# KikeM/romtime

Hardware: AMD Instinct MI355X
Metric: snapshot-DoF/s for POD build (higher is better)
Workload: dtype f64

## Files before the change

include/romtime_hip.h:

```cpp
#ifndef ROMTIME_HIP_H
#define ROMTIME_HIP_H

#include <stdint.h>

#ifdef __cplusplus
extern "C" {
#endif

typedef struct rt_ctx rt_ctx;

#define RT_OK 0
#define RT_ERR_ARG (-1)
#define RT_ERR_HIP (-2)
#define RT_ERR_UNSUPPORTED (-3)
#define RT_WARN_ZERO_NORM 1
#define RT_WARN_SINGULAR 2

#define RT_ROW_MAJOR 0
#define RT_COL_MAJOR 1

int rt_version(void);
int rt_ctx_create(rt_ctx** out, int device);
void rt_ctx_destroy(rt_ctx* ctx);
int rt_ctx_set_stream(rt_ctx* ctx, void* hip_stream);
// ... 113 lines not shown

int rt_trajectory_errors(rt_ctx* ctx, const double* B, int64_t ldb, const double* A, int64_t lda, int64_t stride_a,
                         const double* U, int64_t ldu, int u_layout, int64_t stride_u, int64_t N, int64_t k, int64_t nt,
                         int64_t n_traj, double* err, double* ref);

#define RT_FN_POWER 0
int rt_trajectory_integrals(rt_ctx* ctx, const double* E, int64_t lde, const double* w, const double* A, int64_t lda,
                            int64_t stride_a, const double* scale, int64_t n_pts, int64_t k, int64_t nt, int64_t n_traj,
                            int fn, const double* par, double* out);
int rt_trajectory_integrals_plan_info(int num_cus, const double* E, int64_t lde, const double* w, const double* A, int64_t lda,
                                      int64_t stride_a, const double* scale, int64_t n_pts, int64_t k, int64_t nt,
                                      int64_t n_traj, int fn, const double* par, const double* out, int64_t* info3);

int rt_interpolation_errors(rt_ctx* ctx, const double* Psi, int64_t ldpsi, const int64_t* idx, int64_t m, const double* F,
                            int64_t ldf, int f_layout, int64_t N, int64_t S, int64_t group, int64_t pin_row, double pin_value,
                            double* err, double* ref);
int rt_interpolation_errors_plan_info(int num_cus, const double* Psi, int64_t ldpsi, const int64_t* idx, int64_t m,
                                      const double* F, int64_t ldf, int f_layout, int64_t N, int64_t S, int64_t group,
                                      int64_t pin_row, double pin_value, const double* err, const double* ref, int64_t* info3);

#define RT_P1_MASS 0
#define RT_P1_STIFFNESS 1
#define RT_P1_CONVECTION 2
#define RT_P1_TRILINEAR 3
#define RT_P1_LOAD 4
#define RT_P1_LOAD_P2 5
int rt_p1_local_assembly(rt_ctx* ctx, int kind, int64_t nx, const int64_t* rows, const int64_t* cols, int64_t m,
                         int64_t n_states, const double* h, const double* coef, int state_mode, const double* state,
                         double* out);

int rt_sym_eig_values(rt_ctx* ctx, const double* G, int64_t n, double* lam, int* status);
int rt_sym_eig_values_part(rt_ctx* ctx, const double* G, int64_t n, int64_t first, int64_t count, double* lam,
                           int* status);
int rt_sym_eig_vectors(rt_ctx* ctx, int64_t n, int64_t k, const double* lam, double* W);

int rt_sym_jacobi_eigh(rt_ctx* ctx, const double* A, int64_t n, double* lam, double* W, int max_sweeps, int* sweeps_done,
                       int* status);

int rt_host_jacobi_eigh(double* A, int64_t n, double* W, double* lam, int max_sweeps, int* sweeps_done);

int rt_bench_mfma_f64(rt_ctx* ctx, int iters, double* tflops);
int rt_bench_copy(rt_ctx* ctx, void* dst, const void* src, int64_t bytes, int reps, double* gbps);

#ifdef __cplusplus
}
#endif
#endif
```

romtime_amd/_lib.py:

```python
from __future__ import annotations

import ctypes as C
import os
import threading
import weakref

_HERE = os.path.dirname(os.path.abspath(__file__))
LIB_PATH = os.path.join(_HERE, "lib", "libromtime_hip.so")

ROW_MAJOR, COL_MAJOR = 0, 1
RT_OK = 0
WARN_ZERO_NORM, WARN_SINGULAR = 1, 2

_p = C.c_void_p
_i64 = C.c_int64
_int = C.c_int

SOLVER_DIRECT, SOLVER_GMRES = 0, 1


class GmresOpts(C.Structure):

    _fields_ = [("rtol", C.c_double), ("atol", C.c_double), ("restart", _i64), ("maxiter", _i64)]

# ... 17 lines not shown
    "rt_last_sweep_stats": (_int, [_p, C.POINTER(_i64)]),
    "rt_gram": (_int, [_p, _p, _i64, _i64, _i64, _int, _p]),
    "rt_gram_scale": (_int, [_p, _p, _i64, _p, _int, _p]),
    "rt_pod_backproject_weights": (_int, [_p, _p, _i64, _i64, _p, _p, _p]),
    "rt_pod_enqueue": (_int, [_p, _p, _i64, _i64, _i64, _int, _i64, _int, _p, _p, _p, _p, _p, _p, _p]),
    "rt_pod_orth": (_int, [_p, _p, _i64, _i64, _i64, _int, _i64, C.c_double, _int, _p, _i64, C.POINTER(_i64), _p, _p,
                           C.POINTER(_int)]),
    "rt_gemm_tn": (_int, [_p, _p, _i64, _int, _p, _i64, _int, _i64, _i64, _i64, _p, _i64]),
    "rt_gemm_nn": (_int, [_p, _p, _i64, _int, _p, _i64, _i64, _i64, _i64, _p, _i64, _int]),
    "rt_rank_update": (_int, [_p, _p, _i64, _p, _p, _i64, _p, _i64, _i64, _i64, _i64, C.c_double, _p, _i64]),
    "rt_gemm_nn_axpby": (_int, [_p, _p, _i64, _int, _p, _i64, _i64, _i64, _i64, C.c_double, C.c_double, _p, _i64, _int]),
    "rt_transpose": (_int, [_p, _p, _i64, _i64, _i64, _p, _i64]),
    "rt_deim_greedy": (_int, [_p, _p, _i64, _i64, _i64, _int, _p, _p, _p]),
    "rt_csr_spmm": (_int, [_p, _p, _p, _p, _i64, _p, _i64, _i64, _p, _i64]),
    "rt_project_csr": (_int, [_p, _p, _p, _p, _i64, _p, _i64, _i64, _p]),
    "rt_project_csr_batched": (_int, [_p, _p, _p, _p, _i64, _int, _i64, _i64, _p, _i64, _i64, _p]),
    "rt_dense_solve_batched": (_int, [_p, _p, _p, _i64, _i64, _p]),
    "rt_dense_solve_multi": (_int, [_p, _p, _i64, _p, _p, _i64, _p]),
    "rt_tracked_solve_batched": (_int, [_p, _p, _p, _p, _i64, _i64, _int, _p]),
    "rt_gmres_batched": (_int, [_p, _p, _p, _p, _i64, _i64, C.POINTER(GmresOpts), _p, _p]),
    "rt_ctx_set_reduced_solver": (_int, [_p, _int, C.POINTER(GmresOpts)]),
    "rt_rom_bdf_sweep": (_int, [_p, _p, _p]),
    "rt_hrom_bdf_sweep": (_int, [_p, _p, _p]),
    "rt_trajectory_errors": (_int, [_p, _p, _i64, _p, _i64, _i64, _p, _i64, _int, _i64, _i64, _i64, _i64, _i64, _p, _p]),
    "rt_trajectory_integrals": (_int, [_p, _p, _i64, _p, _p, _i64, _i64, _p, _i64, _i64, _i64, _i64, _int, C.POINTER(C.c_double), _p]),
    "rt_trajectory_integrals_plan_info": (_int, [_int, _p, _i64, _p, _p, _i64, _i64, _p, _i64, _i64, _i64, _i64, _int,
                                                 C.POINTER(C.c_double), _p, C.POINTER(_i64)]),
    "rt_interpolation_errors": (_int, [_p, _p, _i64, C.POINTER(_i64), _i64, _p, _i64, _int, _i64, _i64, _i64, _i64, C.c_double, _p, _p]),
    "rt_interpolation_errors_plan_info": (_int, [_int, _p, _i64, C.POINTER(_i64), _i64, _p, _i64, _int, _i64, _i64, _i64, _i64,
                                                 C.c_double, _p, _p, C.POINTER(_i64)]),
    "rt_p1_local_assembly": (_int, [_p, _int, _i64, _p, _p, _i64, _i64, _p, _p, _int, _p, _p]),
    "rt_sym_eig_values": (_int, [_p, _p, _i64, _p, _p]),
    "rt_sym_eig_values_part": (_int, [_p, _p, _i64, _i64, _i64, _p, _p]),
    "rt_sym_eig_vectors": (_int, [_p, _i64, _i64, _p, _p]),
    "rt_sym_jacobi_eigh": (_int, [_p, _p, _i64, _p, _p, _int, C.POINTER(_int), _p]),
    "rt_host_jacobi_eigh": (_int, [_p, _i64, _p, _p, _int, C.POINTER(_int)]),
    "rt_bench_mfma_f64": (_int, [_p, _int, C.POINTER(C.c_double)]),
    "rt_bench_copy": (_int, [_p, _p, _p, _i64, _int, C.POINTER(C.c_double)]),
}



class SweepDesc(C.Structure):

    _fields_ = [("N", _i64), ("nnz", _i64), ("r", _i64), ("n_mu", _i64), ("nt", _i64), ("dt", C.c_double),
                ("bdf2", _int), ("indptr", _p), ("indices", _p), ("V", _p), ("mass_values", _p), ("n_terms", _i64),
                ("term_values", _p), ("term_coef", _p), ("tril_values", _p), ("n_rhs", _i64), ("rhs_terms", _p),
                ("rhs_coef", _p)]


class HSweepDesc(C.Structure):

    _fields_ = [("r", _i64), ("n_mu", _i64), ("nt", _i64), ("dt", C.c_double), ("bdf2", _int), ("m_mass", _i64),
                ("m_lin", _i64), ("m_nl", _i64), ("m_rhs", _i64), ("Z", _p), ("Zf", _p), ("F_mass", _p), ("F_lin", _p),
                ("F_rhs", _p), ("W", _p), ("C_nl", _p), ("S_nl", _p)]


_lib = None
_lock = threading.Lock()


class RomtimeHipError(RuntimeError):
    pass


def load():
# ... 156 lines not shown
```

romtime_amd/csrc/api.hip:

```cpp
#include "common.h"

#include <chrono>
#include <new>

namespace {

int grow(rt_ctx* ctx, void** buf, size_t* have, size_t bytes, void** out) {
  if (bytes > *have) {
    RT_HIP_CHECK(ctx, hipStreamSynchronize(ctx->stream));
    if (*buf) RT_HIP_CHECK(ctx, hipFree(*buf));
    *buf = nullptr;
    *have = 0;
    const size_t want = (bytes + ((size_t)1 << 20) - 1) & ~(((size_t)1 << 20) - 1);
    RT_HIP_CHECK(ctx, hipMalloc(buf, want));
    *have = want;
  }
  *out = *buf;
  return RT_OK;
}

__global__ void gram_scale_kernel(double* __restrict__ G, int n, double* __restrict__ colnorm, int normalize,
                                  int* status_flag) {
  const long idx = (long)blockIdx.x * blockDim.x + threadIdx.x;
  if (idx >= (long)n * n) return;
// ... 123 lines not shown
  for (const void* f : ctx->lds_done)
    if (f == fn) return RT_OK;
  RT_HIP_CHECK(ctx, hipFuncSetAttribute(fn, hipFuncAttributeMaxDynamicSharedMemorySize, bytes));
  ctx->lds_done.push_back(fn);
  return RT_OK;
}

int rt_profile_begin(rt_ctx* ctx, bool also_gram) {
  if (!ctx->profile) return RT_OK;
  if (!ctx->ev0) {
    RT_HIP_CHECK(ctx, hipEventCreate(&ctx->ev0));
    RT_HIP_CHECK(ctx, hipEventCreate(&ctx->ev1));
  }
  if (also_gram && !ctx->gev0) {
    RT_HIP_CHECK(ctx, hipEventCreate(&ctx->gev0));
    RT_HIP_CHECK(ctx, hipEventCreate(&ctx->gev1));
  }
  RT_HIP_CHECK(ctx, hipEventRecord(ctx->ev0, ctx->stream));
  if (also_gram) RT_HIP_CHECK(ctx, hipEventRecord(ctx->gev0, ctx->stream));
  return RT_OK;
}

int rt_profile_end(rt_ctx* ctx, bool also_gram) {
  if (!ctx->profile) return RT_OK;
  RT_HIP_CHECK(ctx, hipEventRecord(ctx->ev1, ctx->stream));
  if (also_gram) RT_HIP_CHECK(ctx, hipEventRecord(ctx->gev1, ctx->stream));
  ctx->ev_valid = true;
  if (also_gram) ctx->gev_valid = true;
  return RT_OK;
}

extern "C" {

int rt_version(void) { return 380; }

int rt_ctx_create(rt_ctx** out, int device) {
  if (!out) return RT_ERR_ARG;
  *out = nullptr;
  int count = 0;
  if (hipGetDeviceCount(&count) != hipSuccess || device < 0 || device >= count) return RT_ERR_HIP;
  if (hipSetDevice(device) != hipSuccess) return RT_ERR_HIP;
  rt_ctx* ctx = new (std::nothrow) rt_ctx();
  if (!ctx) return RT_ERR_HIP;
  ctx->device = device;
  hipDeviceProp_t prop;
  if (hipGetDeviceProperties(&prop, device) == hipSuccess) ctx->num_cus = ctx->device_cus = prop.multiProcessorCount;
  if (hipMalloc(reinterpret_cast<void**>(&ctx->dev_counters), sizeof(long) * RT_N_COUNTERS) != hipSuccess ||
      hipMemset(ctx->dev_counters, 0, sizeof(long) * RT_N_COUNTERS) != hipSuccess) {
    delete ctx;
    return RT_ERR_HIP;
  }
  *out = ctx;
  return RT_OK;
}

void rt_ctx_destroy(rt_ctx* ctx) {
  if (!ctx) return;
  (void)hipSetDevice(ctx->device);
  (void)hipDeviceSynchronize();
  if (ctx->scratch) (void)hipFree(ctx->scratch);
  if (ctx->scratch2) (void)hipFree(ctx->scratch2);
  if (ctx->dev_counters) (void)hipFree(ctx->dev_counters);
  if (ctx->gram_pace) (void)hipFree(ctx->gram_pace);
  if (ctx->ev0) (void)hipEventDestroy(ctx->ev0);
  if (ctx->ev1) (void)hipEventDestroy(ctx->ev1);
  if (ctx->gev0) (void)hipEventDestroy(ctx->gev0);
  if (ctx->gev1) (void)hipEventDestroy(ctx->gev1);
// ... 292 lines not shown
```

romtime_amd/csrc/symeig.hip:

```cpp
#include <type_traits>

#include "common.h"
#include "wave_ops.h"

namespace {

constexpr int TW_SMALL = 32;
constexpr int SLOT0 = 160;
constexpr int TW_LARGE = 128;
constexpr int LPR = 64;
constexpr int TT = 1024;
static_assert(LPR == 64, "row reductions use the whole-wave DPP sum");
constexpr int NMAX = 1024;
constexpr int VEC_ITERS = 2;

struct TriParams {
  const double* G;
  double* V;
  double* P;
  double* tau;
  double* d;
  double* e;
  int* flags;
  int n;
// ... 282 lines not shown
      if (gi > k && gi < n) {
        double* row = A + (size_t)li * n;
        const double vi = sv[gi], wi = sw[gi];
        for (int j = k + 1 + tx; j < n; j += LPR) row[j] -= vi * sw[j] + wi * sv[j];
      }
    }
  }
  __syncthreads();
  if (wg == (n - 2) % TW && tid == 0) {
    p.d[n - 2] = sl[n - 2];
    p.e[n - 2] = sl[n - 1];
  }
  if (wg == (n - 1) % TW && tid == 0) {
    p.d[n - 1] = A[(size_t)((n - 1) / TW) * lda + (n - 1)];
    p.e[n - 1] = 0.0;
  }
}

__device__ __forceinline__ double fast_rcp(double q) {
  const double r = __builtin_amdgcn_rcp(q);
  return fma(fma(-q, r, 1.0), r, r);
}

__global__ void symeig_init_kernel(int* flags, double* tau, int n) {
  for (int i = threadIdx.x; i < SLOT0 + TW_LARGE; i += blockDim.x) flags[i] = 0;
  for (int i = threadIdx.x; i < n; i += blockDim.x) tau[i] = 0.0;
}

constexpr int BIS_NS = 2;
template <int NM>
__global__ __launch_bounds__(256) void symeig_bisect_kernel(const double* __restrict__ d, const double* __restrict__ e,
                                                            int n, int first, int count, double* __restrict__ lam,
                                                            const int* flags, int* status, long* counters) {
  if (blockIdx.x == 0 && threadIdx.x == 0) {
    if (status) *status = flags[3];
    if (flags[3]) atomicAdd(reinterpret_cast<unsigned long long*>(&counters[RT_CNT_EIG_TIMEOUT]), 1ull);
  }
  __shared__ double sd[NM], se2[NM];
  __shared__ int s_first[2][4];
  const int tid = threadIdx.x, lane = tid & 63, wid = tid >> 6, half = wid & 1;
  double glo = 1e300, ghi = -1e300, emax = 0.0;
  for (int i = lane; i < n; i += 64) {
    const double di = d[i], ei = (i + 1 < n) ? e[i] : 0.0, el = (i > 0) ? fabs(e[i - 1]) : 0.0;
    sd[i] = di;
    se2[i] = ei * ei;
    glo = fmin(glo, di - el - fabs(ei));
    ghi = fmax(ghi, di + el + fabs(ei));
    emax = fmax(emax, ei * ei);
  }
  glo = rtw::wave_min(glo);
  ghi = rtw::wave_max(ghi);
  emax = rtw::wave_max(emax);
  __syncthreads();
  const double tn = fmax(fabs(glo), fabs(ghi));
  double lo = glo - 2.2e-16 * tn * n - 1e-300, hi = ghi + 2.2e-16 * tn * n + 1e-300;
  const double pivmin = 2.2250738585072014e-308 * fmax(1.0, emax);
  const int j = first + min(2 * (int)blockIdx.x + (wid >> 1), count - 1);
  const int want = n - j;
  constexpr int NSH = 128 * BIS_NS;
  constexpr int NSEC = NSH + 1;
  for (int pass = 0; pass < 7; ++pass) {
    const double h = (hi - lo) / NSEC;
    const int s0 = BIS_NS * (64 * half + lane);
    const double x0 = lo + h * (s0 + 1), x1 = x0 + h;
    double q0 = sd[0] - x0, q1 = sd[0] - x1;
    if (fabs(q0) < pivmin) q0 = -pivmin;
    if (fabs(q1) < pivmin) q1 = -pivmin;
// ... 364 lines not shown
        p.d[n - 1] = p.A[(size_t)(n - 1) * lda + (n - 1)] - (v[q] * w[q] + w[q] * v[q]);
      }
  }
}
static_assert(NWIDE % WIDE_CHUNK == 0 && NWIDE % WIDE_T == 0, "the reflector kernel covers a padded row with PER elements per thread");

template <int LO, int HI, class F>
int size_class(int64_t n, F&& f) {
  if constexpr (LO < HI)
    if (n > LO) return size_class<2 * LO, HI>(n, f);
  return f(std::integral_constant<int, LO>{});
}

struct EigArena {
  void* base;
  double *V, *own, *tau, *d, *e;
  int* flags;
  int carve(rt_ctx* ctx, int64_t n, size_t own_bytes) {
    rt_carver a;
    const size_t oV = a.add(sizeof(double) * n * n), oO = a.add(own_bytes), oT = a.add(sizeof(double) * n),
                 oD = a.add(sizeof(double) * n), oE = a.add(sizeof(double) * n), oF = a.add(sizeof(int) * (SLOT0 + TW_LARGE));
    RT_TRY(rt_scratch2(ctx, a.total(), &base));
    V = a.at<double>(base, oV); own = a.at<double>(base, oO);
    tau = a.at<double>(base, oT); d = a.at<double>(base, oD);
    e = a.at<double>(base, oE); flags = a.at<int>(base, oF);
    return RT_OK;
  }
  void publish(rt_ctx* ctx, int64_t n) const {
    ctx->eig.d = d; ctx->eig.e = e; ctx->eig.V = V; ctx->eig.tau = tau; ctx->eig.n = n; ctx->eig.base = base;
    ctx->eig.gen = ctx->scratch2_gen;
  }
};

int launch_bisect(rt_ctx* ctx, const EigArena& a, int64_t n, int64_t first, int64_t count, double* lam, int* status) {
  return size_class<512, NWIDE>(n, [&](auto nm) {
    hipLaunchKernelGGL(symeig_bisect_kernel<decltype(nm)::value>, dim3((unsigned)((count + 1) / 2)), dim3(256), 0, ctx->stream, a.d,
                       a.e, (int)n, (int)first, (int)count, lam, a.flags, status, ctx->dev_counters);
    RT_HIP_CHECK(ctx, hipGetLastError());
    return (int)RT_OK;
  });
}

}

static int sym_eig_values_wide(rt_ctx* ctx, const double* G, int64_t n, int64_t first, int64_t count, double* lam,
                               int* status) {
  const int lda = (int)((n + WIDE_CHUNK - 1) / WIDE_CHUNK * WIDE_CHUNK);
  const size_t nvec = (size_t)3 * (lda + WIDE_ROWS) + (size_t)(n + WIDE_ROWS);
  static_assert(sizeof(double) * WIDE_CHUNK % 256 == 0, "the vector buffers start on a 256-byte boundary");
  const size_t cells = (size_t)(n + WIDE_ROWS) * lda;
  EigArena ar;
  RT_TRY(ar.carve(ctx, n, sizeof(double) * (cells + nvec)));
  WideParams wp;
  wp.V = ar.V; wp.A = ar.own;
  wp.vb = wp.A + cells; wp.w = wp.vb + (size_t)2 * (lda + WIDE_ROWS);
  wp.pr = wp.w + (lda + WIDE_ROWS);
  wp.tau = ar.tau; wp.d = ar.d; wp.e = ar.e;
  wp.n = (int)n; wp.lda = lda; wp.counters = ctx->dev_counters;
  hipStream_t st = ctx->stream;
  hipLaunchKernelGGL(symeig_init_kernel, dim3(1), dim3(256), 0, st, ar.flags, wp.tau, (int)n);
  hipLaunchKernelGGL(symeig_wide_load_kernel, dim3((unsigned)((cells + WIDE_T - 1) / WIDE_T)), dim3(WIDE_T), 0, st, G, wp,
                     (long)nvec);
  hipLaunchKernelGGL(symeig_wide_reflect_kernel, dim3(1), dim3(WIDE_T), 0, st, wp, -1);
  RT_HIP_CHECK(ctx, hipGetLastError());
  for (int k = 0; k + 2 < (int)n; ++k) {
    const int rows = (int)n - 1 - k;
    hipLaunchKernelGGL(symeig_wide_sweep_kernel, dim3((unsigned)((rows + WIDE_ROWS - 1) / WIDE_ROWS)), dim3(WIDE_T), 0, st, wp, k);
    hipLaunchKernelGGL(symeig_wide_reflect_kernel, dim3(1), dim3(WIDE_T), 0, st, wp, k);
  }
  RT_HIP_CHECK(ctx, hipGetLastError());
  RT_TRY(launch_bisect(ctx, ar, n, first, count, lam, status));
  ar.publish(ctx, n);
  return RT_OK;
}

extern "C" int rt_sym_eig_values(rt_ctx* ctx, const double* G, int64_t n, double* lam, int* status) {
  return rt_sym_eig_values_part(ctx, G, n, 0, n, lam, status);
}

extern "C" int rt_sym_eig_values_part(rt_ctx* ctx, const double* G, int64_t n, int64_t first, int64_t count, double* lam,
                                      int* status) {
  if (!ctx) return RT_ERR_ARG;
  RT_ARG_CHECK(ctx, G && lam && n >= 3 && first >= 0 && count >= 1 && first + count <= n);
  if (n > NWIDE) {
    ctx->err = "rt_sym_eig_values: n > 2048 not supported (the limit of the device eigensolver)";
    return RT_ERR_UNSUPPORTED;
  }
  if (n > NMAX) return sym_eig_values_wide(ctx, G, n, first, count, lam, status);
  const bool large = n > 512;
  const bool small_team = !large && ctx->num_cus < TW_SMALL && ctx->num_cus >= TW_SMALL / 2;
  int tw = large ? TW_LARGE : (small_team ? TW_SMALL / 2 : TW_SMALL);
  const bool local = n <= 64;
  if (local) tw = 1;
  if (tw > ctx->num_cus) {
    ctx->err = "rt_sym_eig_values: not enough compute units for the cooperative tridiagonalisation";
    return RT_ERR_UNSUPPORTED;
  }
  EigArena ar;
  RT_TRY(ar.carve(ctx, n, sizeof(double) * 4 * n));
  TriParams tp;
  tp.G = G; tp.n = (int)n; tp.tw = tw;
  tp.spread = (!large && !local && ctx->eig_one_xcd && ctx->num_cus / 8 >= tw) ? 1 : 0;
  tp.local = local ? 1 : 0;
  tp.xcd = ctx->eig_xcd & 7;
  tp.V = ar.V; tp.P = ar.own; tp.tau = ar.tau; tp.d = ar.d; tp.e = ar.e; tp.flags = ar.flags;
  tp.counters = ctx->dev_counters;
  hipStream_t st = ctx->stream;
  hipLaunchKernelGGL(symeig_init_kernel, dim3(1), dim3(256), 0, st, tp.flags, tp.tau, (int)n);

  const int RB = (int)((n + tw - 1) / tw);
  const size_t lds = sizeof(double) * ((size_t)RB * (local ? n + 2 : n) + 5 * n + 16);
  const auto tridiag = [&](auto nm) -> int {
    const auto kernel = &symeig_tridiag_kernel<decltype(nm)::value>;
    RT_TRY(rt_func_lds(ctx, reinterpret_cast<const void*>(kernel), 150 * 1024));
    int per_cu = 0;
    RT_HIP_CHECK(ctx, hipOccupancyMaxActiveBlocksPerMultiprocessor(&per_cu, kernel, TT, lds));
    if ((long)per_cu * ctx->num_cus < tw) {
      ctx->err = "rt_sym_eig_values: the device cannot keep all cooperating workgroups resident";
      return RT_ERR_UNSUPPORTED;
    }
    hipLaunchKernelGGL(kernel, dim3(tp.spread ? 16 * tw : tw), dim3(TT), lds, st, tp);
    RT_HIP_CHECK(ctx, hipGetLastError());
    return RT_OK;
  };
  RT_TRY((size_class<128, NMAX>(n, tridiag)));
  RT_TRY(launch_bisect(ctx, ar, n, first, count, lam, status));
  ar.publish(ctx, n);
  return RT_OK;
}

extern "C" int rt_sym_eig_vectors(rt_ctx* ctx, int64_t n, int64_t k, const double* lam, double* W) {
  if (!ctx) return RT_ERR_ARG;
  RT_ARG_CHECK(ctx, lam && W && k >= 1 && k <= n);
  if (ctx->eig.n != n || ctx->eig.base == nullptr || ctx->eig.base != ctx->scratch2 || ctx->eig.gen != ctx->scratch2_gen) {
    ctx->err = "rt_sym_eig_vectors: must follow rt_sym_eig_values on the same ctx and matrix with no other composite "
               "operator (greedy, projection, sweep) in between";
    return RT_ERR_ARG;
  }
  VecParams vp;
  vp.d = ctx->eig.d; vp.e = ctx->eig.e; vp.lam = lam; vp.V = ctx->eig.V; vp.tau = ctx->eig.tau;
  vp.W = W; vp.n = (int)n; vp.k = (int)k;
  const int nblk = (int)((n - 2 + RBK - 1) / RBK);
  void* cbuf = nullptr;
  int rc = rt_scratch(ctx, sizeof(double) * 6 * (size_t)nblk, &cbuf);
  if (rc != RT_OK) return rc;
  vp.C = static_cast<const double*>(cbuf);
  return size_class<128, NWIDE>(n, [&](auto nm) -> int {
    constexpr int NM = decltype(nm)::value;
    const size_t vlds = sizeof(double) * (8 * NM + 8) + NM;
    RT_TRY(rt_func_lds(ctx, reinterpret_cast<const void*>(&symeig_vectors_kernel<NM>), (NM > 1024 ? 136 : 80) * 1024));
    hipLaunchKernelGGL(symeig_wy_kernel<NM>, dim3((unsigned)nblk), dim3(64), 0, ctx->stream, vp.V, (int)n,
                       static_cast<double*>(cbuf));
    hipLaunchKernelGGL(symeig_vectors_kernel<NM>, dim3((unsigned)k), dim3(64), vlds, ctx->stream, vp);
    RT_HIP_CHECK(ctx, hipGetLastError());
    return RT_OK;
  });
}
```

romtime_amd/ops.py:

```python
from __future__ import annotations

import ctypes as C

import numpy as np
import torch

from . import _lib, pod_rules
from ._lib import COL_MAJOR, ROW_MAJOR, Context, RomtimeHipError

_p = C.c_void_p


def _ptr(t):
    return _p(t.data_ptr()) if t is not None else _p(None)


def _need_gpu():
    if not torch.cuda.is_available():
        raise RomtimeHipError("no MI355X visible: romtime_amd's hot path runs on the GPU only (there is no CPU fallback)")


def to_device(a, device=None) -> torch.Tensor:
    _need_gpu()
    if isinstance(a, torch.Tensor):
# ... 378 lines not shown
    mode, st = 0, None
    if state is not None:
        st = to_device(state).contiguous()
        width = 2 * nx + 1 if kind == "load_p2" else nx + 1
        if tuple(st.shape) != (n_states, width):
            raise RomtimeHipError(f"p1_local_assembly: `state` must be (n_states, {width}) for kind {kind!r}")
        mode = 1
    elif ramp is not None:
        st = to_device(np.atleast_1d(ramp) if not isinstance(ramp, torch.Tensor) else ramp).contiguous()
        mode = 2
    elif poly is not None:
        st = to_device(poly).contiguous()
        if tuple(st.shape) != (n_states, 3):
            raise RomtimeHipError("p1_local_assembly: `poly` must be (n_states, 3)")
        mode = 3
    out = torch.empty((n_states, m), dtype=torch.float64, device=h.device)
    ctx.check(ctx.lib.rt_p1_local_assembly(ctx.handle, P1_KINDS[kind], int(nx), _ptr(rows), _ptr(cols), m, n_states, _ptr(h),
                                           _ptr(coef), mode, _ptr(st), _ptr(out)), "rt_p1_local_assembly")
    return out


def sym_eig_values(G: torch.Tensor, first: int = 0, count: int | None = None):
    ctx = Context.current()
    n = G.shape[0]
    assert G.is_contiguous() and G.shape == (n, n)
    count = n - first if count is None else count
    lam = torch.empty(n, dtype=torch.float64, device=G.device)
    status = torch.zeros(1, dtype=torch.int32, device=G.device)
    ctx.check(ctx.lib.rt_sym_eig_values_part(ctx.handle, _ptr(G), n, first, count, _ptr(lam), _ptr(status)),
              "rt_sym_eig_values_part")
    return lam, status


def sym_eig_vectors(lam: torch.Tensor, k: int, first: int = 0) -> torch.Tensor:
    ctx = Context.current()
    n = lam.numel()
    W = torch.empty((n, k), dtype=torch.float64, device=lam.device)
    ctx.check(ctx.lib.rt_sym_eig_vectors(ctx.handle, n, k, _ptr(lam[first:]), _ptr(W)), "rt_sym_eig_vectors")
    return W


def sym_jacobi_eigh(G: torch.Tensor, max_sweeps: int = 60):
    ctx = Context.current()
    n = G.shape[0]
    if G.dtype != torch.float64 or not G.is_cuda or G.dim() != 2 or G.shape != (n, n):
        raise RomtimeHipError("sym_jacobi_eigh: expected a square float64 CUDA tensor")
    G = G.contiguous()
    lam = torch.empty(n, dtype=torch.float64, device=G.device)
    W = torch.empty((n, n), dtype=torch.float64, device=G.device)
    status = torch.zeros(1, dtype=torch.int32, device=G.device)
    sweeps = C.c_int(0)
    ctx.check(ctx.lib.rt_sym_jacobi_eigh(ctx.handle, _ptr(G), n, _ptr(lam), _ptr(W), int(max_sweeps), C.byref(sweeps),
                                         _ptr(status)), "rt_sym_jacobi_eigh")
    if sweeps.value >= max_sweeps and int(status.item()) != 0:
        import warnings

        warnings.warn(f"romtime_amd: sym_jacobi_eigh stopped at max_sweeps = {max_sweeps} with rotations still applied",
                      RuntimeWarning)
    return lam, W, int(sweeps.value)


def transpose(src: torch.Tensor) -> torch.Tensor:
    ctx = Context.current()
    src = src.contiguous()
    rows, cols = src.shape
    dst = torch.empty((cols, rows), dtype=torch.float64, device=src.device)
# ... 19 lines not shown
```

romtime_amd/pipeline.py:

```python
from __future__ import annotations

import collections
import ctypes as C
import os
import weakref

import torch

from . import _lib, ops, pod, pod_rules

_p = C.c_void_p


SMALL_SET = 150_000_000
_STREAMS: dict = {}
_STREAMS_PID: list = []
_OPEN_RUNS = weakref.WeakSet()


def shutdown():
    import gc

    if not _STREAMS:
        return
    if _STREAMS_PID and _STREAMS_PID[0] != os.getpid():
        _STREAMS.clear()
        return
    try:
        for gen in list(_OPEN_RUNS):
            gen.close()
        torch.cuda.synchronize()
        gc.collect()
        torch.cuda.empty_cache()
        lib = _lib.load()
        _lib.Context.unbind_streams()
        for st in list(_STREAMS.values()):
            lib.rt_stream_destroy(_p(st.cuda_stream))
    finally:
        _STREAMS.clear()


def _masked_stream(lib, dev, first, count):
    key = (dev, first, count)
    if key not in _STREAMS:
        h = _p()
        rc = lib.rt_stream_create_cu_range(dev, first, count, C.byref(h))
        if rc != 0:
# ... 66 lines not shown
    def _gram(self, item):
        X = item["X"]
        n = X.shape[1]
        with self.ctxG.use(self.sG):
            item["t0"] = torch.cuda.Event(enable_timing=True)
            item["t0"].record()
            Gbuf = torch.empty(n * n + 1, dtype=torch.float64, device=X.device)
            item["G"] = ops.gram(X, out=Gbuf[: n * n].view(n, n))
            Gbuf[n * n:].fill_(float(X.shape[0]))
            item["k0"] = torch.cuda.Event(enable_timing=True)
            item["k0"].record()
            item["Gbuf"] = Gbuf
        st = self.sG if self.sR is None else self.sR
        with torch.cuda.stream(st):
            if st is not self.sG:
                st.wait_event(item["k0"])
            if self.group is not None:
                import torch.distributed as dist

                dist.all_reduce(Gbuf, op=dist.ReduceOp.SUM, group=self.group)
            item["g"] = torch.cuda.Event(enable_timing=True)
            item["g"].record()

    def _eig(self, item):
        k, normalize = item["k"], item["normalize"]
        item["owner"] = item["index"] % self.world
        if self.rank != item["owner"]:
            return
        with self.ctxE.use(self.sE):
            self.sE.wait_event(item["g"])
            G = item["G"]
            n = G.shape[0]
            colnorm, flag = ops.gram_scale(G, normalize)
            lam_d, status = ops.sym_eig_values(G)
            Z = ops.sym_eig_vectors(lam_d, k)
            Zs = ops.backproject_weights(Z, lam_d, colnorm if normalize else None)
            item["payload"] = torch.cat([lam_d, colnorm, status.to(torch.float64), flag.to(torch.float64), Zs.reshape(-1)])
            item["_keep"] = (lam_d, status, flag, Z, Zs, colnorm)
            item["ec"] = torch.cuda.Event(enable_timing=True)
            item["ec"].record()

    def _share(self, item):
        n, k = item["G"].shape[0], item["k"]
        st = self.sE if self.group_e is None else self.sC
        with torch.cuda.stream(st):
            if self.group_e is not None:
                import torch.distributed as dist

                if self.rank == item["owner"]:
                    st.wait_event(item["ec"])
                else:
                    item["payload"] = torch.empty(n * (k + 2) + 2, dtype=torch.float64, device=item["G"].device)
                dist.broadcast(item["payload"], src=dist.get_global_rank(self.group_e, item["owner"]), group=self.group_e)
            payload = item["payload"]
            item["colnorm"].copy_(payload[n:2 * n])
            item["Zs"] = payload[2 * n + 2:].view(n, k)
            head = pod.pack_head(payload[:n], payload[2 * n:2 * n + 2], item["Gbuf"][-1:])
            item["head"] = torch.empty(head.numel(), dtype=torch.float64).pin_memory()
            item["head"].copy_(head, non_blocking=True)
            item["_keep2"] = head
            item["e"] = torch.cuda.Event(enable_timing=True)
            item["e"].record()

    def _backproject(self, item):
        ctx, st = self.ctxG, self.sG
        with ctx.use(st):
            st.wait_event(item["e"])
            ops.gemm_nn(item["X"], item["Zs"], out=item["Q"])
            item["b"] = torch.cuda.Event(enable_timing=True)
            item["b"].record()

    def _regular(self, item):
        self.recomputed += 1
        self.sE.synchronize()
        return pod.pod_device(item["X"], num=item["num"], normalize=item["normalize"], group=self.group)

    def _finish(self, item):
        if item["direct"]:
            return self._regular(item)
        item["b"].synchronize()
        head = pod_rules.parse_head(item["head"].numpy(), item["X"].shape[1])
        if item["normalize"] and head.zero_norm:
            raise pod_rules.zero_norm_error()
        r = pod_rules.single_pass_rank(head.lam, head.status, head.n_rows, item["k"], num=item["num"])
        self.last_stage_ms = dict(gram_kernel_ms=item["t0"].elapsed_time(item["k0"]),
                                  gram_allreduce_ms=item["t0"].elapsed_time(item["g"]),
                                  eig_chain_ms=item["g"].elapsed_time(item["e"]),
                                  gram_start_to_basis_ms=item["t0"].elapsed_time(item["b"]))
        self.gram_kernel_ms.append(self.last_stage_ms["gram_kernel_ms"])
        if r is None:
            return self._regular(item)
        s = pod_rules.sigma(head.lam)
        return dict(Q=item["Q"], s=s, energy=pod_rules.energy(s), VT=None, r=r, passes=1, colnorm=item["colnorm"])

    def run(self, snapshot_sets, num, normalize=True, depth=2):
        if not num:
            raise ValueError("PodPipeline enqueues ahead of the spectrum: it needs `num` (pod.py:51-53)")
        gen = self._run(snapshot_sets, num, normalize, depth)
        _OPEN_RUNS.add(gen)
        return gen

    def _run(self, snapshot_sets, num, normalize, depth):
        main = torch.cuda.current_stream(self.device)
        flight = collections.deque()
        it = iter(snapshot_sets)
        self._admitted = 0
        depth = max(depth, self.world + 1)
        streams = [st for st in (self.sG, self.sE, self.sC) if st is not None]
        materialised = isinstance(snapshot_sets, (list, tuple))
        if materialised:
            _wait_for(streams, main)

        def admit():
            try:
                X = _checked(next(it), self)
            except StopIteration:
                return None
            item = dict(X=X, num=num, k=int(min(num, X.shape[1])), normalize=bool(normalize), index=self._admitted)
            self._admitted += 1
            n = X.shape[1]
            rows = X.shape[0] * self.world
            item["direct"] = not (3 <= n <= 512) or rows * n < self.small_set
            if not item["direct"]:
                item["Q"] = torch.empty((X.shape[0], item["k"]), dtype=torch.float64, device=X.device)
                item["colnorm"] = torch.empty(n, dtype=torch.float64, device=X.device)
                if not materialised:
                    _wait_for(streams, main)
                self._gram(item)
                self._eig(item)
            return item

        pending = collections.deque()
        for _ in range(self.world):
            item = admit()
            if item is None:
                break
            pending.append(item)
        while pending:
            cur = pending.popleft()
            if not cur["direct"]:
                self._share(cur)
            nxt = admit()
            if nxt is not None:
                pending.append(nxt)
            if not cur["direct"]:
                self._backproject(cur)
            flight.append(cur)
            while len(flight) > depth or (not pending and flight):
                yield self._finish(flight.popleft())
        for st in streams:
            _wait_for([main], st)

    def map(self, snapshot_sets, num, normalize=True, depth=2):
        return list(self.run(snapshot_sets, num, normalize=normalize, depth=depth))


class PodLanes:

    def __init__(self, lanes: int = 8, device=None):
        if not torch.cuda.is_available():
            raise _lib.RomtimeHipError("no MI355X visible: romtime_amd's hot path runs on the GPU only")
        if not (1 <= int(lanes) <= 8):
            raise ValueError("lanes must be 1 .. 8 (one per XCD)")
        self.device = torch.device("cuda", torch.cuda.current_device() if device is None else device)
        self.ctx, self.streams = [], []
        for lane in range(int(lanes)):
            c = _lib.Context(self.device.index)
            c.set_option("eig_xcd", lane)
            self.ctx.append(c)
            self.streams.append(torch.cuda.Stream(self.device))
        self.recomputed = 0

    def close(self):
        torch.cuda.synchronize(self.device)

    def _enqueue(self, item, lane):
        X, k, normalize = item["X"], item["k"], item["normalize"]
        with self.ctx[lane].use(self.streams[lane]):
            Q, lam_d, status2, colnorm, keep = ops.pod_enqueue(X, k, normalize)
            head = pod.pack_head(lam_d, status2)
            item["head"] = torch.empty(head.numel(), dtype=torch.float64).pin_memory()
            item["head"].copy_(head, non_blocking=True)
            item["Q"], item["colnorm"] = Q, colnorm
            item["_keep"] = (keep, head, lam_d, status2)
            item["done"] = torch.cuda.Event()
            item["done"].record()

# ... 146 lines not shown
```

romtime_amd/csrc/sweep.hip:

```cpp
#include "common.h"
#include "sweep_step.h"

namespace {

constexpr int EX_KP = 144, EX_SA = EX_KP + 2, EX_SB = 34, EX_THREADS = 256;
constexpr int EX_LA = 64 * EX_KP / 2 / EX_THREADS;
constexpr int EX_LB = EX_KP * 32 / 2 / EX_THREADS;

__global__ __launch_bounds__(EX_THREADS) void expansion_kernel(const double* __restrict__ G, long ldg,
                                                                const double* __restrict__ Z, long ldz,
                                                                double* __restrict__ Cm, long ldc, int R, int K, long N) {
  extern __shared__ __attribute__((aligned(16))) double ex_sm[];
  double* sA = ex_sm;
  double* sB = ex_sm + 64 * EX_SA;
  const int tid = threadIdx.x, lane = tid & 63, l15 = lane & 15, l4 = lane >> 4;
  const int wid = __builtin_amdgcn_readfirstlane(tid >> 6);
  const long n0 = (long)blockIdx.x * 32;
  d4 acc[2][2] = {{d4{0, 0, 0, 0}, d4{0, 0, 0, 0}}, {d4{0, 0, 0, 0}, d4{0, 0, 0, 0}}};
  d2 ra[EX_LA], rb[EX_LB];
  auto fetch = [&](int k0) {
#pragma unroll
    for (int i = 0; i < EX_LA; ++i) {
      const int q = tid + EX_THREADS * i, row = q / (EX_KP / 2), kk = 2 * (q % (EX_KP / 2));
      const int k = k0 + kk;
// ... 46 lines not shown
    for (int c = 0; c < 4; ++c) {
      const int row = 16 * wid + l4 + 4 * c;
      const long col = n0 + 16 * j + l15;
      if (row < R && col < N) Cm[(long)row * ldc + col] = acc[j][0][c] + acc[j][1][c];
    }
}

}

int rt_expansion_gemm(rt_ctx* ctx, const double* G, long ldg, const double* Z, long ldz, double* Cm, long ldc, long R,
                      long K, long N) {
  if (R > 64 || R < 1 || K < 2 || N < 2 || ((K | N | ldg | ldz) & 1) ||
      ((reinterpret_cast<size_t>(G) | reinterpret_cast<size_t>(Z)) & 15))
    return RT_ERR_UNSUPPORTED;
  const size_t lds = sizeof(double) * (64 * EX_SA + EX_KP * EX_SB);
  const dim3 grid((unsigned)((N + 31) / 32));
  RT_TRY(rt_func_lds(ctx, reinterpret_cast<const void*>(&expansion_kernel), (int)lds));
  hipLaunchKernelGGL(expansion_kernel, grid, dim3(EX_THREADS), lds, ctx->stream, G, ldg, Z, ldz, Cm, ldc, (int)R, (int)K, N);
  RT_HIP_CHECK(ctx, hipGetLastError());
  ctx->last_grid = grid.x; ctx->last_splits = 1; ctx->last_tile = 64 * 1000 + 32;
  return RT_OK;
}

namespace {

__global__ void sweep_rows_kernel(const long* __restrict__ indptr, long N, int* __restrict__ row_of) {
  const long row = (long)blockIdx.x * blockDim.x + threadIdx.x;
  if (row >= N) return;
  for (long e = indptr[row]; e < indptr[row + 1]; ++e) row_of[e] = (int)row;
}

constexpr int SV_QMAX = 8;
constexpr long SV_LDS_BYTES = 32 * 1024;
template <bool COEF_LDS>
__global__ __launch_bounds__(256) void sweep_values_kernel(const double* __restrict__ mass,
                                                           const double* __restrict__ terms, int Q,
                                                           const double* __restrict__ coef,
                                                           const double* __restrict__ tril,
                                                           const int* __restrict__ row_of,
                                                           const double* __restrict__ uh,
                                                           const double* __restrict__ uhp, int extrapolate, long nnz,
                                                           long N, int B, double bdf, double dt,
                                                           double* __restrict__ kval) {
  extern __shared__ double s_coef[];
  if (COEF_LDS) {
    for (int i = threadIdx.x; i < B * Q; i += blockDim.x) s_coef[i] = coef[i];
    __syncthreads();
  }
  const long e = (long)blockIdx.x * blockDim.x + threadIdx.x;
  if (e >= nnz) return;
  double tq[SV_QMAX];
#pragma unroll
  for (int q = 0; q < SV_QMAX; ++q) tq[q] = (q < Q) ? terms[(long)q * nnz + e] : 0.0;
  const double m = bdf * mass[e];
  const double tv = tril ? tril[e] : 0.0;
  const long row = tril ? row_of[e] : 0;
#pragma unroll 4
  for (int b = 0; b < B; ++b) {
    double s = 0.0;
#pragma unroll
    for (int q = 0; q < SV_QMAX; ++q)
      if (q < Q) s = fma(COEF_LDS ? s_coef[b * Q + q] : coef[b * Q + q], tq[q], s);
    for (int q = SV_QMAX; q < Q; ++q)
      s = fma(COEF_LDS ? s_coef[b * Q + q] : coef[b * Q + q], terms[(long)q * nnz + e], s);
    if (tril) {
      const double u = uh[(long)b * N + row];
      const double us = extrapolate ? 2.0 * u - uhp[(long)b * N + row] : u;
      s = fma(us, tv, s);
    }
    kval[(long)b * nnz + e] = fma(dt, s, m);
  }
}

__global__ void hsweep_advance_kernel(const double* __restrict__ x, int do_store, int r, const rt_advance a) {
  extern __shared__ double su[];
  hsweep_advance_rows(a, blockIdx.x, r, x, do_store, su, threadIdx.x, blockDim.x);
}

__global__ void hsweep_count_kernel(long* ctr) { *ctr += 1; }

__global__ void step_rhs_kernel(const rt_step_rhs rq, int r, double* __restrict__ rhs) {
  extern __shared__ double su[];
  const int b = blockIdx.x, t = threadIdx.x;
  if (t < r) su[t] = step_rhs_state(rq, b, r, t);
  __syncthreads();
  if (t < r) rhs[(long)b * r + t] = step_rhs_row(rq, step_rhs_mn(rq, b, r), step_rhs_forcing_rows(rq, b), r, t, su);
}

struct StepWork {
  double* KN;
  double* rhs;
  double* un;
  double* unm1;
  double* Xinv;
  int* info;
  double* gwork;
};

int step_work_get(rt_ctx* ctx, long r, long B, long kn_mats, size_t extra, StepWork* w, char** extra_base) {
  rt_carver a;
  const bool gmres = ctx->reduced_solver == RT_SOLVER_GMRES;
  const size_t oKN = a.add(sizeof(double) * kn_mats * r * r), oRhs = a.add(sizeof(double) * B * r),
               oUn = a.add(sizeof(double) * B * r), oUm = a.add(sizeof(double) * B * r),
// ... 38 lines not shown

  rt_carver a;
  const size_t oRow = a.add(sizeof(int) * nnz), oMN = a.add(sizeof(double) * r * r), oFN = a.add(sizeof(double) * (F ? F : 1) * r),
               oUh = a.add(sizeof(double) * B * N), oUp = a.add(sizeof(double) * B * N), oXT = a.add(sizeof(double) * r * B),
               oKv = a.add(sizeof(double) * B * nnz), oTab = a.add(rt_project_stage_table_bytes(N));
  StepWork w;
  char* b8 = nullptr;
  int rc = step_work_get(ctx, r, B, B, a.total(), &w, &b8);
  if (rc != RT_OK) return rc;
  int* row_of = a.at<int>(b8, oRow);
  double *MN = a.at<double>(b8, oMN), *fN = a.at<double>(b8, oFN), *uh = a.at<double>(b8, oUh), *uhp = a.at<double>(b8, oUp),
         *xT = a.at<double>(b8, oXT), *kval = a.at<double>(b8, oKv);
  void* stage_table = a.at<void>(b8, oTab);

  RT_HIP_CHECK(ctx, hipMemsetAsync(uh, 0, sizeof(double) * B * N, st));
  RT_HIP_CHECK(ctx, hipMemsetAsync(uhp, 0, sizeof(double) * B * N, st));
  hipLaunchKernelGGL(sweep_rows_kernel, dim3((unsigned)((N + 255) / 256)), dim3(256), 0, st,
                     reinterpret_cast<const long*>(d->indptr), N, row_of);
  RT_HIP_CHECK(ctx, hipGetLastError());
  rc = rt_project_stage_table(ctx, d->indptr, d->indices, N, stage_table);
  if (rc != RT_OK) return rc;
  int banded = -1;
  rc = rt_project_stage_table_banded(ctx, stage_table, &banded);
  if (rc != RT_OK) return rc;
  rc = rt_project_fused(ctx, d->indptr, d->indices, d->mass_values, 1, 0, 1, N, d->V, r, r, MN, stage_table, banded);
  if (rc != RT_OK) return rc;
  if (F) {
    rc = rt_gemm_strided(ctx, d->rhs_terms, 1, N, d->V, r, 1, N, F, r, fN, r, 1, false, true);
    if (rc != RT_OK) return rc;
  }

  for (long step = 0; step < nt; ++step) {
    const bool second = d->bdf2 && step > 0;
    if ((long)sizeof(double) * B * Q <= SV_LDS_BYTES)
      hipLaunchKernelGGL(sweep_values_kernel<true>, dim3((unsigned)((nnz + 255) / 256)), dim3(256), sizeof(double) * B * Q,
                         st, d->mass_values, d->term_values, Q, Q ? d->term_coef + step * B * Q : nullptr, d->tril_values,
                         row_of, uh, uhp, d->bdf2 ? 1 : 0, nnz, N, (int)B, second ? 1.5 : 1.0, d->dt, kval);
    else
      hipLaunchKernelGGL(sweep_values_kernel<false>, dim3((unsigned)((nnz + 255) / 256)), dim3(256), 0, st,
                         d->mass_values, d->term_values, Q, d->term_coef + step * B * Q, d->tril_values, row_of, uh, uhp,
                         d->bdf2 ? 1 : 0, nnz, N, (int)B, second ? 1.5 : 1.0, d->dt, kval);
    RT_HIP_CHECK(ctx, hipGetLastError());
    rc = rt_project_fused(ctx, d->indptr, d->indices, kval, 1, nnz, B, N, d->V, r, r, w.KN, stage_table, banded);
    if (rc != RT_OK) return rc;
    const double c0 = d->bdf2 ? 2.0 : 1.0, c1 = d->bdf2 ? -0.5 : 0.0;
    rt_step_rhs rq{MN, w.un, w.unm1, c0, c1, d->dt, F ? d->rhs_coef + step * B * F : nullptr, fN, F};
    rq.mn_stride = 0;
    rt_advance close{};
    close.un = w.un; close.unm1 = w.unm1; close.out = uN_out; close.step_done = step; close.nt = nt;
    close.keep_prev = d->bdf2 ? 1 : 0; close.do_coef = 0; close.xT = xT; close.B = (int)B; close.enabled = 1;
    rc = sweep_step_solve(ctx, w, r, B, step > 0 ? 1 : 0, rq, close);
    if (rc != RT_OK) return rc;
    double* tmp = uhp; uhp = uh; uh = tmp;
    rc = rt_gemm_nn(ctx, d->V, r, RT_ROW_MAJOR, xT, B, N, r, B, uh, N, RT_COL_MAJOR);
    if (rc != RT_OK) return rc;
  }
  return RT_OK;
}

extern "C" int rt_hrom_bdf_sweep(rt_ctx* ctx, const rt_hsweep_desc* d, double* uN_out) {
  if (!ctx) return RT_ERR_ARG;
  RT_ARG_CHECK(ctx, d && uN_out);
  RT_ARG_CHECK(ctx, d->r >= 1 && d->r <= 128 && d->n_mu >= 1 && d->nt >= 1);
  RT_ARG_CHECK(ctx, d->m_mass >= 1 && d->m_lin >= 0 && d->m_nl >= 0 && d->m_rhs >= 0 && d->Z && d->F_mass);
  RT_ARG_CHECK(ctx, (d->m_lin == 0 || d->F_lin) && (d->m_nl == 0 || d->W) && (d->m_rhs == 0 || (d->Zf && d->F_rhs)));
  const long r = d->r, B = d->n_mu, nt = d->nt, mm = d->m_mass, ml = d->m_lin, mn = d->m_nl, mf = d->m_rhs;
  const long M = mm + ml + mn, rr = r * r;
  hipStream_t st = ctx->stream;
  const bool gmres = ctx->reduced_solver == RT_SOLVER_GMRES;
  const size_t g_bytes = (sizeof(double) * 2 * B * M + 255) / 256 * 256;
  StepWork w;
  char* b8 = nullptr;
// ... 82 lines not shown
```

Before: 91.11 billion.

## Split eigenvalue bisection so backprojection starts after leading k eigenpairs

On a single device, the pipeline now bisects only the leading k eigenvalues before computing eigenvectors and weights. It records a weights-ready event so the backprojection GEMM can start early. The remaining eigenvalues are bisected afterwards via a new rt_sym_eig_values_more entry point that reuses the held tridiagonal. The run loop also admits more items ahead (lag) to overlap stages across snapshot sets. This adds a new API with an ordering precondition and keeps more buffers in flight.

```diff
diff --git a/include/romtime_hip.h b/include/romtime_hip.h
--- a/include/romtime_hip.h
+++ b/include/romtime_hip.h
@@ -169,6 +169,7 @@
 int rt_sym_eig_values(rt_ctx* ctx, const double* G, int64_t n, double* lam, int* status);
 int rt_sym_eig_values_part(rt_ctx* ctx, const double* G, int64_t n, int64_t first, int64_t count, double* lam,
                            int* status);
+int rt_sym_eig_values_more(rt_ctx* ctx, int64_t n, int64_t first, int64_t count, double* lam);
 int rt_sym_eig_vectors(rt_ctx* ctx, int64_t n, int64_t k, const double* lam, double* W);
 
 int rt_sym_jacobi_eigh(rt_ctx* ctx, const double* A, int64_t n, double* lam, double* W, int max_sweeps, int* sweeps_done,
diff --git a/romtime_amd/_lib.py b/romtime_amd/_lib.py
--- a/romtime_amd/_lib.py
+++ b/romtime_amd/_lib.py
@@ -73,6 +73,7 @@
     "rt_p1_local_assembly": (_int, [_p, _int, _i64, _p, _p, _i64, _i64, _p, _p, _int, _p, _p]),
     "rt_sym_eig_values": (_int, [_p, _p, _i64, _p, _p]),
     "rt_sym_eig_values_part": (_int, [_p, _p, _i64, _i64, _i64, _p, _p]),
+    "rt_sym_eig_values_more": (_int, [_p, _i64, _i64, _i64, _p]),
     "rt_sym_eig_vectors": (_int, [_p, _i64, _i64, _p, _p]),
     "rt_sym_jacobi_eigh": (_int, [_p, _p, _i64, _p, _p, _int, C.POINTER(_int), _p]),
     "rt_host_jacobi_eigh": (_int, [_p, _i64, _p, _p, _int, C.POINTER(_int)]),
diff --git a/romtime_amd/csrc/api.hip b/romtime_amd/csrc/api.hip
--- a/romtime_amd/csrc/api.hip
+++ b/romtime_amd/csrc/api.hip
@@ -179,7 +179,7 @@
 
 extern "C" {
 
-int rt_version(void) { return 380; }
+int rt_version(void) { return 390; }
 
 int rt_ctx_create(rt_ctx** out, int device) {
   if (!out) return RT_ERR_ARG;
diff --git a/romtime_amd/csrc/symeig.hip b/romtime_amd/csrc/symeig.hip
--- a/romtime_amd/csrc/symeig.hip
+++ b/romtime_amd/csrc/symeig.hip
@@ -338,7 +338,7 @@
 __global__ __launch_bounds__(256) void symeig_bisect_kernel(const double* __restrict__ d, const double* __restrict__ e,
                                                             int n, int first, int count, double* __restrict__ lam,
                                                             const int* flags, int* status, long* counters) {
-  if (blockIdx.x == 0 && threadIdx.x == 0) {
+  if (flags && blockIdx.x == 0 && threadIdx.x == 0) {
     if (status) *status = flags[3];
     if (flags[3]) atomicAdd(reinterpret_cast<unsigned long long*>(&counters[RT_CNT_EIG_TIMEOUT]), 1ull);
   }
@@ -769,13 +769,18 @@
   }
 };
 
-int launch_bisect(rt_ctx* ctx, const EigArena& a, int64_t n, int64_t first, int64_t count, double* lam, int* status) {
+int launch_bisect(rt_ctx* ctx, const double* d, const double* e, const int* flags, int64_t n, int64_t first, int64_t count,
+                  double* lam, int* status) {
   return size_class<512, NWIDE>(n, [&](auto nm) {
-    hipLaunchKernelGGL(symeig_bisect_kernel<decltype(nm)::value>, dim3((unsigned)((count + 1) / 2)), dim3(256), 0, ctx->stream, a.d,
-                       a.e, (int)n, (int)first, (int)count, lam, a.flags, status, ctx->dev_counters);
+    hipLaunchKernelGGL(symeig_bisect_kernel<decltype(nm)::value>, dim3((unsigned)((count + 1) / 2)), dim3(256), 0, ctx->stream, d,
+                       e, (int)n, (int)first, (int)count, lam, flags, status, ctx->dev_counters);
     RT_HIP_CHECK(ctx, hipGetLastError());
     return (int)RT_OK;
   });
+}
+
+bool eig_held(const rt_ctx* ctx, int64_t n) {
+  return ctx->eig.n == n && ctx->eig.base != nullptr && ctx->eig.base == ctx->scratch2 && ctx->eig.gen == ctx->scratch2_gen;
 }
 
 }
@@ -806,7 +811,7 @@
     hipLaunchKernelGGL(symeig_wide_reflect_kernel, dim3(1), dim3(WIDE_T), 0, st, wp, k);
   }
   RT_HIP_CHECK(ctx, hipGetLastError());
-  RT_TRY(launch_bisect(ctx, ar, n, first, count, lam, status));
+  RT_TRY(launch_bisect(ctx, ar.d, ar.e, ar.flags, n, first, count, lam, status));
   ar.publish(ctx, n);
   return RT_OK;
 }
@@ -861,15 +866,27 @@
     return RT_OK;
   };
   RT_TRY((size_class<128, NMAX>(n, tridiag)));
-  RT_TRY(launch_bisect(ctx, ar, n, first, count, lam, status));
+  RT_TRY(launch_bisect(ctx, ar.d, ar.e, ar.flags, n, first, count, lam, status));
   ar.publish(ctx, n);
   return RT_OK;
+}
+
+extern "C" int rt_sym_eig_values_more(rt_ctx* ctx, int64_t n, int64_t first, int64_t count, double* lam) {
+  if (!ctx) return RT_ERR_ARG;
+  RT_ARG_CHECK(ctx, lam && n >= 3 && n <= NWIDE && first >= 0 && count >= 0 && first + count <= n);
+  if (!eig_held(ctx, n)) {
+    ctx->err = "rt_sym_eig_values_more: must follow rt_sym_eig_values[_part] on the same ctx and an n x n matrix with no "
+               "other composite operator (greedy, projection, sweep) in between";
+    return RT_ERR_ARG;
+  }
+  if (count == 0) return RT_OK;
+  return launch_bisect(ctx, ctx->eig.d, ctx->eig.e, nullptr, n, first, count, lam, nullptr);
 }
 
 extern "C" int rt_sym_eig_vectors(rt_ctx* ctx, int64_t n, int64_t k, const double* lam, double* W) {
   if (!ctx) return RT_ERR_ARG;
   RT_ARG_CHECK(ctx, lam && W && k >= 1 && k <= n);
-  if (ctx->eig.n != n || ctx->eig.base == nullptr || ctx->eig.base != ctx->scratch2 || ctx->eig.gen != ctx->scratch2_gen) {
+  if (!eig_held(ctx, n)) {
     ctx->err = "rt_sym_eig_vectors: must follow rt_sym_eig_values on the same ctx and matrix with no other composite "
                "operator (greedy, projection, sweep) in between";
     return RT_ERR_ARG;
diff --git a/romtime_amd/ops.py b/romtime_amd/ops.py
--- a/romtime_amd/ops.py
+++ b/romtime_amd/ops.py
@@ -434,6 +434,15 @@
     return lam, status
 
 
+def sym_eig_values_more(lam: torch.Tensor, first: int, count: int | None = None) -> torch.Tensor:
+    ctx = Context.current()
+    n = lam.numel()
+    assert lam.is_contiguous() and lam.dtype == torch.float64
+    count = n - first if count is None else count
+    ctx.check(ctx.lib.rt_sym_eig_values_more(ctx.handle, n, first, count, _ptr(lam)), "rt_sym_eig_values_more")
+    return lam
+
+
 def sym_eig_vectors(lam: torch.Tensor, k: int, first: int = 0) -> torch.Tensor:
     ctx = Context.current()
     n = lam.numel()
diff --git a/romtime_amd/pipeline.py b/romtime_amd/pipeline.py
--- a/romtime_amd/pipeline.py
+++ b/romtime_amd/pipeline.py
@@ -13,6 +13,7 @@
 
 
 SMALL_SET = 150_000_000
+LAG = 3
 _STREAMS: dict = {}
 _STREAMS_PID: list = []
 _OPEN_RUNS = weakref.WeakSet()
@@ -145,13 +146,21 @@
             G = item["G"]
             n = G.shape[0]
             colnorm, flag = ops.gram_scale(G, normalize)
-            lam_d, status = ops.sym_eig_values(G)
+            split = self.group_e is None
+            lam_d, status = ops.sym_eig_values(G, 0, k if split else n)
             Z = ops.sym_eig_vectors(lam_d, k)
             Zs = ops.backproject_weights(Z, lam_d, colnorm if normalize else None)
+            if split:
+                item["Zs"] = Zs
+                item["w"] = torch.cuda.Event(enable_timing=True)
+                item["w"].record()
+                ops.sym_eig_values_more(lam_d, k)
             item["payload"] = torch.cat([lam_d, colnorm, status.to(torch.float64), flag.to(torch.float64), Zs.reshape(-1)])
             item["_keep"] = (lam_d, status, flag, Z, Zs, colnorm)
             item["ec"] = torch.cuda.Event(enable_timing=True)
             item["ec"].record()
+        if split:
+            self._share(item)
 
     def _share(self, item):
         n, k = item["G"].shape[0], item["k"]
@@ -167,18 +176,20 @@
                 dist.broadcast(item["payload"], src=dist.get_global_rank(self.group_e, item["owner"]), group=self.group_e)
             payload = item["payload"]
             item["colnorm"].copy_(payload[n:2 * n])
-            item["Zs"] = payload[2 * n + 2:].view(n, k)
+            if self.group_e is not None:
+                item["Zs"] = payload[2 * n + 2:].view(n, k)
             head = pod.pack_head(payload[:n], payload[2 * n:2 * n + 2], item["Gbuf"][-1:])
             item["head"] = torch.empty(head.numel(), dtype=torch.float64).pin_memory()
             item["head"].copy_(head, non_blocking=True)
             item["_keep2"] = head
             item["e"] = torch.cuda.Event(enable_timing=True)
             item["e"].record()
+            item.setdefault("w", item["e"])
 
     def _backproject(self, item):
         ctx, st = self.ctxG, self.sG
         with ctx.use(st):
-            st.wait_event(item["e"])
+            st.wait_event(item["w"])
             ops.gemm_nn(item["X"], item["Zs"], out=item["Q"])
             item["b"] = torch.cuda.Event(enable_timing=True)
             item["b"].record()
@@ -192,6 +203,7 @@
         if item["direct"]:
             return self._regular(item)
         item["b"].synchronize()
+        item["e"].synchronize()
         head = pod_rules.parse_head(item["head"].numpy(), item["X"].shape[1])
         if item["normalize"] and head.zero_norm:
             raise pod_rules.zero_norm_error()
@@ -199,6 +211,7 @@
         self.last_stage_ms = dict(gram_kernel_ms=item["t0"].elapsed_time(item["k0"]),
                                   gram_allreduce_ms=item["t0"].elapsed_time(item["g"]),
                                   eig_chain_ms=item["g"].elapsed_time(item["e"]),
+                                  weights_ready_ms=item["g"].elapsed_time(item["w"]),
                                   gram_start_to_basis_ms=item["t0"].elapsed_time(item["b"]))
         self.gram_kernel_ms.append(self.last_stage_ms["gram_kernel_ms"])
         if r is None:
@@ -206,19 +219,25 @@
         s = pod_rules.sigma(head.lam)
         return dict(Q=item["Q"], s=s, energy=pod_rules.energy(s), VT=None, r=r, passes=1, colnorm=item["colnorm"])
 
-    def run(self, snapshot_sets, num, normalize=True, depth=2):
+    def run(self, snapshot_sets, num, normalize=True, depth=2, lag=LAG):
         if not num:
             raise ValueError("PodPipeline enqueues ahead of the spectrum: it needs `num` (pod.py:51-53)")
-        gen = self._run(snapshot_sets, num, normalize, depth)
+        if int(lag) < 1:
+            raise ValueError("lag must be at least 1")
+        gen = self._run(snapshot_sets, num, normalize, depth, int(lag))
         _OPEN_RUNS.add(gen)
         return gen
 
-    def _run(self, snapshot_sets, num, normalize, depth):
+    def _run(self, snapshot_sets, num, normalize, depth, lag):
         main = torch.cuda.current_stream(self.device)
         flight = collections.deque()
         it = iter(snapshot_sets)
         self._admitted = 0
-        depth = max(depth, self.world + 1)
+        if self.group_e is not None:
+            lag = 1
+        ahead = max(self.world, lag)
+        depth = max(depth, ahead + 1)
+        done = depth - lag + 1
         streams = [st for st in (self.sG, self.sE, self.sC) if st is not None]
         materialised = isinstance(snapshot_sets, (list, tuple))
         if materialised:
@@ -244,14 +263,14 @@
             return item
 
         pending = collections.deque()
-        for _ in range(self.world):
+        for _ in range(ahead):
             item = admit()
             if item is None:
                 break
             pending.append(item)
         while pending:
             cur = pending.popleft()
-            if not cur["direct"]:
+            if not cur["direct"] and self.group_e is not None:
                 self._share(cur)
             nxt = admit()
             if nxt is not None:
@@ -259,13 +278,13 @@
             if not cur["direct"]:
                 self._backproject(cur)
             flight.append(cur)
-            while len(flight) > depth or (not pending and flight):
+            while len(flight) > done or (not pending and flight):
                 yield self._finish(flight.popleft())
         for st in streams:
             _wait_for([main], st)
 
-    def map(self, snapshot_sets, num, normalize=True, depth=2):
-        return list(self.run(snapshot_sets, num, normalize=normalize, depth=depth))
+    def map(self, snapshot_sets, num, normalize=True, depth=2, lag=LAG):
+        return list(self.run(snapshot_sets, num, normalize=normalize, depth=depth, lag=lag))
 
 
 class PodLanes:
```

Result: no change. 91.41 billion (median of 4 runs) (+0.3%).

## Split sweep_values kernel over groups of batch columns with XCD-aware block mapping

Applied to the files above, without the earlier changes.

The per-step value kernel now assigns each block a group of 8 batch columns instead of looping over all B, so the grid grows by ceil(B/8). Block indices are remapped so blocks that share the same nnz range but handle different batch groups land on the same XCD, which aims at L2 reuse of the terms, mass and tril loads. Within a group the batch loop is fully unrolled with independent accumulators to add memory-level parallelism, and stores use nontemporal hints. In exchange, the per-entry loads (terms, mass, tril, row_of) are repeated once per group, and LDS coefficient staging now covers only the group's 8 rows.

```diff
diff --git a/romtime_amd/csrc/sweep.hip b/romtime_amd/csrc/sweep.hip
--- a/romtime_amd/csrc/sweep.hip
+++ b/romtime_amd/csrc/sweep.hip
@@ -102,6 +102,12 @@
 
 constexpr int SV_QMAX = 8;
 constexpr long SV_LDS_BYTES = 32 * 1024;
+constexpr int SV_GROUP = 8;
+constexpr int SV_XCDS = 8;
+inline unsigned sweep_values_grid(long nnz, long B) {
+  const long blocks = ((nnz + 255) / 256 + SV_XCDS - 1) / SV_XCDS * SV_XCDS;
+  return (unsigned)(blocks * ((B + SV_GROUP - 1) / SV_GROUP));
+}
 template <bool COEF_LDS>
 __global__ __launch_bounds__(256) void sweep_values_kernel(const double* __restrict__ mass,
                                                            const double* __restrict__ terms, int Q,
@@ -113,11 +119,21 @@
                                                            long N, int B, double bdf, double dt,
                                                            double* __restrict__ kval) {
   extern __shared__ double s_coef[];
+  const int groups = (B + SV_GROUP - 1) / SV_GROUP;
+  const long slot = blockIdx.x / SV_XCDS;
+  const long block = slot / groups * SV_XCDS + blockIdx.x % SV_XCDS;
+  const int b0 = (int)(slot % groups) * SV_GROUP;
+  int bj[SV_GROUP];
+#pragma unroll
+  for (int j = 0; j < SV_GROUP; ++j) bj[j] = b0 + j < B ? b0 + j : B - 1;
   if (COEF_LDS) {
-    for (int i = threadIdx.x; i < B * Q; i += blockDim.x) s_coef[i] = coef[i];
+    for (int i = threadIdx.x; i < SV_GROUP * Q; i += blockDim.x) {
+      const int j = i / Q;
+      s_coef[i] = coef[(b0 + j < B ? b0 + j : B - 1) * Q + (i - j * Q)];
+    }
     __syncthreads();
   }
-  const long e = (long)blockIdx.x * blockDim.x + threadIdx.x;
+  const long e = block * 256 + threadIdx.x;
   if (e >= nnz) return;
   double tq[SV_QMAX];
 #pragma unroll
@@ -125,20 +141,33 @@
   const double m = bdf * mass[e];
   const double tv = tril ? tril[e] : 0.0;
   const long row = tril ? row_of[e] : 0;
-#pragma unroll 4
-  for (int b = 0; b < B; ++b) {
-    double s = 0.0;
-#pragma unroll
-    for (int q = 0; q < SV_QMAX; ++q)
-      if (q < Q) s = fma(COEF_LDS ? s_coef[b * Q + q] : coef[b * Q + q], tq[q], s);
-    for (int q = SV_QMAX; q < Q; ++q)
-      s = fma(COEF_LDS ? s_coef[b * Q + q] : coef[b * Q + q], terms[(long)q * nnz + e], s);
-    if (tril) {
-      const double u = uh[(long)b * N + row];
-      const double us = extrapolate ? 2.0 * u - uhp[(long)b * N + row] : u;
-      s = fma(us, tv, s);
-    }
-    kval[(long)b * nnz + e] = fma(dt, s, m);
+  double us[SV_GROUP];
+  if (tril) {
+#pragma unroll
+    for (int j = 0; j < SV_GROUP; ++j) us[j] = uh[(long)bj[j] * N + row];
+    if (extrapolate) {
+#pragma unroll
+      for (int j = 0; j < SV_GROUP; ++j) us[j] = 2.0 * us[j] - uhp[(long)bj[j] * N + row];
+    }
+  }
+  double s[SV_GROUP];
+#pragma unroll
+  for (int j = 0; j < SV_GROUP; ++j) s[j] = 0.0;
+#pragma unroll
+  for (int q = 0; q < SV_QMAX; ++q)
+    if (q < Q) {
+#pragma unroll
+      for (int j = 0; j < SV_GROUP; ++j) s[j] = fma(COEF_LDS ? s_coef[j * Q + q] : coef[bj[j] * Q + q], tq[q], s[j]);
+    }
+  for (int q = SV_QMAX; q < Q; ++q) {
+    const double t = terms[(long)q * nnz + e];
+#pragma unroll
+    for (int j = 0; j < SV_GROUP; ++j) s[j] = fma(COEF_LDS ? s_coef[j * Q + q] : coef[bj[j] * Q + q], t, s[j]);
+  }
+#pragma unroll
+  for (int j = 0; j < SV_GROUP; ++j) {
+    if (tril) s[j] = fma(us[j], tv, s[j]);
+    if (b0 + j < B) __builtin_nontemporal_store(fma(dt, s[j], m), &kval[(long)(b0 + j) * nnz + e]);
   }
 }
 
@@ -243,12 +272,12 @@
 
   for (long step = 0; step < nt; ++step) {
     const bool second = d->bdf2 && step > 0;
-    if ((long)sizeof(double) * B * Q <= SV_LDS_BYTES)
-      hipLaunchKernelGGL(sweep_values_kernel<true>, dim3((unsigned)((nnz + 255) / 256)), dim3(256), sizeof(double) * B * Q,
+    if ((long)sizeof(double) * (B > SV_GROUP ? B : SV_GROUP) * Q <= SV_LDS_BYTES)
+      hipLaunchKernelGGL(sweep_values_kernel<true>, dim3(sweep_values_grid(nnz, B)), dim3(256), sizeof(double) * SV_GROUP * Q,
                          st, d->mass_values, d->term_values, Q, Q ? d->term_coef + step * B * Q : nullptr, d->tril_values,
                          row_of, uh, uhp, d->bdf2 ? 1 : 0, nnz, N, (int)B, second ? 1.5 : 1.0, d->dt, kval);
     else
-      hipLaunchKernelGGL(sweep_values_kernel<false>, dim3((unsigned)((nnz + 255) / 256)), dim3(256), 0, st,
+      hipLaunchKernelGGL(sweep_values_kernel<false>, dim3(sweep_values_grid(nnz, B)), dim3(256), 0, st,
                          d->mass_values, d->term_values, Q, d->term_coef + step * B * Q, d->tril_values, row_of, uh, uhp,
                          d->bdf2 ? 1 : 0, nnz, N, (int)B, second ? 1.5 : 1.0, d->dt, kval);
     RT_HIP_CHECK(ctx, hipGetLastError());
```

Measured after the change: 91.59 billion before, 91.76 billion after, median of 2. About the same (+0.2%).
